# taintpro98/rnd-semantic-segmentation

Measured on AMD Instinct MI355X. Metric: train images/sec at 769x769 bf16 (DeepLabV2-ResNet101 + ASPP), higher is better.
Workload: dtype bf16; 1 GPU; train_src.py DeepLabV2-R101 bf16, 769x769 synthetic Cityscapes crops, batch 8 per GPU, 1xMI355X; global_batch=8, parallelism=dp1, weights=formula (synthetic), hip_graph_replay=False

## Files before the change

include/mi355seg.h:

```cpp
#ifndef MI355SEG_H
#define MI355SEG_H

#include <stddef.h>
#include <stdint.h>

#ifdef __cplusplus
extern "C" {
#endif

#define MI355SEG_VERSION 100

#define MI_OK 0
#define MI_EINVAL (-22)
#define MI_ENOMEM (-12)
#define MI_EHIP (-5)

#define MI_EPI_SCALE_BIAS 1
#define MI_EPI_RESIDUAL 2
#define MI_EPI_RELU 4
#define MI_EPI_MASK 8
#define MI_EPI_OUT_F32 16
#define MI_EPI_ZSPLIT 32
#define MI_EPI_WRITE_MASK 64
#define MI_EPI_LEAKY 256
// ... 63 lines not shown
int mi_upsample_ac_fwd(const float* low, float* up, int B, int h, int w, int K, int H, int W, void* stream);
int mi_upsample_ac_bwd(const float* dup, float* dlow, int B, int h, int w, int K, int H, int W, void* stream);

size_t mi_ce_workspace(int B, int H, int W);
int mi_softmax_ce_fwd(const float* logits, const int64_t* labels, float* loss_out ,
                      int B, int K, int H, int W, int ignore_index, void* workspace, size_t workspace_bytes, void* stream);
int mi_softmax_ce_bwd(const float* logits, const int64_t* labels, const float* loss_out, float* dlogits,
                      int B, int K, int H, int W, int ignore_index, float grad_scale, void* stream);

size_t mi_upsample_ce_workspace(int B, int h, int w, int K, int H, int W);
int mi_upsample_ce(const float* low, const int64_t* labels, float* loss_out , float* dlow,
                   int B, int h, int w, int K, int H, int W, int ignore_index, float grad_scale,
                   void* workspace, size_t workspace_bytes, void* stream);

int mi_upsample_ce_ex(const float* low, const int64_t* labels, float* loss_out , float* dlow,
                      int B, int h, int w, int K, int H, int W, int ignore_index, float grad_scale, int align_corners,
                      void* workspace, size_t workspace_bytes, void* stream);

int mi_upsample_softmax(const float* low, float* probs, uint8_t* pred, int B, int h, int w, int K, int H, int W, void* stream);

typedef struct { const float* low; int h, w; int mirror; } MiProbSource;
int mi_upsample_softmax_multi(const MiProbSource* src, int n, float* probs, int K, int H, int W, float div_a, float div_b, void* stream);

int mi_image_resize_ac(const float* x, float* out, int B, int C, int H, int W, int Ho, int Wo, int with_mirror, void* stream);

int mi_sgd_step(float* p, const float* g, float* buf, size_t n, float lr, float momentum, float weight_decay, void* stream);
int mi_sgd_step_dev(float* p, const float* g, float* buf, size_t n, const float* hyper , void* stream);

int mi_stem_pool_fwd(const void* y, const float* scale, const float* shift, void* pool, uint8_t* idx,
                     int B, int Hc, int Wc, int C, int Hp, int Wp, void* stream);
int mi_stem_pool_bwd(const void* dpool, const uint8_t* idx, const float* scale, void* dy,
                     int B, int Hc, int Wc, int C, int Hp, int Wp, void* stream);
int mi_stem_im2col(const void* x_bf16_nhwc, void* col_bf16, int B, int H, int W, int Ho, int Wo, int ncols, void* stream);

int mi_bias_grad_bf16(const void* dy_bf16, float* db, int M, int N, int accumulate,
                      void* workspace , size_t workspace_bytes, void* stream);
size_t mi_upsample_softce_workspace(int B, int h, int w, int K, int H, int W);
int mi_upsample_softce(const float* seg_low, float inv_temperature, float clip, const float* d_low, int ldD, int domain,
                       float* loss_out, float* dd_low, int B, int h, int w, int K, int H, int W, float grad_scale,
                       void* workspace, size_t workspace_bytes, void* stream);
size_t mi_upsample_softce_2grid_workspace(int B, int hd, int wd, int K, int H, int W);
int mi_upsample_softce_2grid(const float* seg_low, int hs, int ws, int seg_align_corners, float inv_temperature, float clip,
                             const float* d_low, int hd, int wd, int ldD, int d_align_corners, int domain, float grad_scale,
                             float* loss_out, float* dd_low, int B, int K, int H, int W, void* workspace, size_t workspace_bytes, void* stream);
int mi_adam_step(float* p, const float* g, float* exp_avg, float* exp_avg_sq, size_t n, float lr, float beta1, float beta2,
                 float eps, int step, void* stream);
int mi_adam_step_clamped(float* p, float* g, float* exp_avg, float* exp_avg_sq, size_t n, float lr, float beta1, float beta2,
                         float eps, int step, float grad_clamp, void* stream);

int mi_adam_step_dev(float* p, float* g, float* exp_avg, float* exp_avg_sq, size_t n, const float* hyper , void* stream);

int mi_pack_weight_f32(const float* w_oihw, float* wp, int O, int I, int ksize, void* stream);
int mi_conv_f32(const float* a, const float* wp, float* out, int B, int Ha, int Wa, int Ca, int Ho, int Wo, int N,
                int ksize, int stride, int pad, int dil, const float* scale, const float* bias, const float* res,
                int flags, void* stream);
int mi_stem_f32(const float* x_nchw, const float* w, const float* scale, const float* shift, float* y_nhwc,
                int B, int H, int W, void* stream);
int mi_maxpool_f32(const float* y_nhwc, float* pool_nhwc, int B, int Hc, int Wc, int C, void* stream);

int mi_comm_unique_id(void* id128 );
int mi_comm_init_rank(void** comm , int nranks, const void* id128 , int rank);
int mi_comm_destroy(void* comm);
int mi_allreduce_bucket(void* ptr, size_t count, int dtype, int average, void* comm, void* stream);

int mi_relu_mask(const void* x_bf16, const void* msk, void* y_bf16, size_t n, int bits, void* stream);
int mi_frozen_bn_fold(const float* w, const float* b, const float* mean, const float* var, float* scale, float* shift, int n, void* stream);
// ... 129 lines not shown
```

rnd_semantic_segmentation_amd/_lib.py:

```python
import ctypes
import os

import torch
from ctypes import c_char_p, c_double, c_float, c_int, c_long, c_size_t, c_void_p

_HERE = os.path.dirname(os.path.abspath(__file__))
LIB_PATH = os.environ.get("MI355SEG_LIB") or os.path.join(_HERE, "libmi355seg.so")
HEADER_PATH = os.path.join(os.path.dirname(_HERE), "include", "mi355seg.h")

P, I, F, Z, L = c_void_p, c_int, c_float, c_size_t, c_long

SIGNATURES = {
    "mi_version": (I, []),
    "mi_last_error": (c_char_p, []),
    "mi_pack_weight_fwd": (I, [P, P, I, I, I, P]),
    "mi_pack_weight_dgrad": (I, [P, P, P, I, I, I, P]),
    "mi_pack_weights_multi": (I, [P, P, P, P, P, I, I, P]),
    "mi_conv_gemm": (I, [P, P, P] + [I] * 12 + [P, P, P, P, P, I, I, F, P]),
    "mi_conv_gemm_route": (I, [I] * 10),
    "mi_conv_gemm_pp": (I, [P, P, P] + [I] * 12 + [P, P, P, P, P, I, I, F, I, P]),
    "mi_conv_chain": (I, [P] * 6 + [L, I, I, I] + [P] * 8 + [I, I, P]),
    "mi_conv_wgrad_workspace": (Z, [I] * 6),
    "mi_conv_wgrad_route": (I, [I] * 12),
    "mi_conv_wgrad": (I, [P, P, P] + [I] * 11 + [P, I, I, I, Z, P, Z, P]),
    "mi_conv_wgrad_job_bytes": (Z, []),
    "mi_conv_wgrad_partial": (I, [P, P, P] + [I] * 11 + [P, I, I, I, Z, P, Z, P, P]),
    "mi_conv_wgrad_reduce": (I, [P, I, P]),
    "mi_aspp_pack_fwd": (I, [P, P, I, I, P]),
    "mi_aspp_pack_dgrad": (I, [P, P, I, I, P]),
    "mi_aspp_col2im": (I, [P, P, P, I, I, I, I, P, P]),
    "mi_aspp_im2col": (I, [P, P, I, I, I, I, P, P]),
    "mi_colsum_workspace": (Z, [I, I]),
    "mi_aspp_bias_grad": (I, [P, P, I, I, I, P, Z, P]),
    "mi_upsample_ac_fwd": (I, [P, P] + [I] * 6 + [P]),
    "mi_upsample_ac_bwd": (I, [P, P] + [I] * 6 + [P]),
    "mi_ce_workspace": (Z, [I, I, I]),
    "mi_softmax_ce_fwd": (I, [P, P, P, I, I, I, I, I, P, Z, P]),
    "mi_softmax_ce_bwd": (I, [P, P, P, P, I, I, I, I, I, F, P]),
    "mi_upsample_ce_workspace": (Z, [I] * 6),
    "mi_upsample_ce": (I, [P, P, P, P] + [I] * 7 + [F, P, Z, P]),
    "mi_upsample_ce_ex": (I, [P, P, P, P] + [I] * 7 + [F, I, P, Z, P]),
    "mi_upsample_softmax": (I, [P, P, P] + [I] * 6 + [P]),
    "mi_upsample_softmax_multi": (I, [P, I, P, I, I, I, F, F, P]),
    "mi_image_resize_ac": (I, [P, P] + [I] * 7 + [P]),
    "mi_stem_pool_fwd": (I, [P, P, P, P, P] + [I] * 6 + [P]),
    "mi_stem_pool_bwd": (I, [P, P, P, P] + [I] * 6 + [P]),
    "mi_stem_im2col": (I, [P, P] + [I] * 6 + [P]),
    "mi_bias_grad_bf16": (I, [P, P, I, I, I, P, Z, P]),
    "mi_upsample_softce_workspace": (Z, [I] * 6),
    "mi_upsample_softce": (I, [P, F, F, P, I, I, P, P] + [I] * 6 + [F, P, Z, P]),
    "mi_upsample_softce_2grid_workspace": (Z, [I] * 6),
    "mi_upsample_softce_2grid": (I, [P, I, I, I, F, F, P, I, I, I, I, I, F, P, P, I, I, I, I, P, Z, P]),
    "mi_adam_step": (I, [P, P, P, P, Z, F, F, F, F, I, P]),
    "mi_adam_step_clamped": (I, [P, P, P, P, Z, F, F, F, F, I, F, P]),
    "mi_adam_step_dev": (I, [P, P, P, P, Z, P, P]),
    "mi_sgd_step": (I, [P, P, P, Z, F, F, F, P]),
    "mi_sgd_step_dev": (I, [P, P, P, Z, P, P]),
    "mi_pack_weight_f32": (I, [P, P, I, I, I, P]),
    "mi_conv_f32": (I, [P, P, P] + [I] * 11 + [P, P, P, I, P]),
    "mi_stem_f32": (I, [P, P, P, P, P, I, I, I, P]),
    "mi_maxpool_f32": (I, [P, P, I, I, I, I, P]),
    "mi_comm_unique_id": (I, [P]),
    "mi_comm_init_rank": (I, [P, I, P, I]),
    "mi_comm_destroy": (I, [P]),
    "mi_allreduce_bucket": (I, [P, Z, I, I, P, P]),
    "mi_relu_mask": (I, [P, P, P, Z, I, P]),
    "mi_frozen_bn_fold": (I, [P, P, P, P, P, P, I, P]),
    "mi_structure_loss_workspace": (Z, [I, I, I]),
    "mi_structure_loss": (I, [P, P, I, I, I, P, P, F, P, Z, P]),
    "mi_bn_workspace": (Z, [L, I]),
    "mi_bn_colsum": (I, [P, P, L, I, P, P, Z, P]),
    "mi_bn_apply": (I, [P, P, P, P, P, P, P, I, L, I, P]),
    "mi_bn_colsum2": (I, [P, P, L, I, P, P, P, Z, P]),
    "mi_conv_gemm_stats_workspace": (Z, [L, I]),
    "mi_conv_gemm_stats": (I, [P, P, P] + [I] * 11 + [P, P, P, Z, P, P, P, P, P, F, F, P, P]),
    "mi_bn_finalize": (I, [P, P, P, c_double, P, P, P, P, P, F, F, P, I, P]),
    "mi_bn_bwd_colsums": (I, [P, P, P, P, P, L, I, P, P, P, Z, P]),
    "mi_bn_bwd_apply": (I, [P, P, P, P, P, P, P, F, P, P, L, I, P]),
    "mi_gconv_pack_elems": (Z, [I] * 4),
    "mi_gconv_pack_multi": (I, [P, P, P, P, I, I, P]),
# ... 84 lines not shown
```

rnd_semantic_segmentation_amd/csrc/stem.hip:

```cpp
#include "mi_common.h"

namespace {

__global__ void stem_pool_fwd_kernel(const bf16x8* __restrict__ y, const float* __restrict__ scale, const float* __restrict__ shift,
                                     bf16x8* __restrict__ pool, uint8_t* __restrict__ idx, int B, int Hc, int Wc, int C8, int Hp, int Wp) {
    const long id = (long)blockIdx.x * blockDim.x + threadIdx.x;
    if (id >= (long)B * Hp * Wp * C8) return;
    const int c8 = (int)(id % C8);
    const int wo = (int)((id / C8) % Wp), ho = (int)((id / ((long)C8 * Wp)) % Hp), b = (int)(id / ((long)C8 * Wp * Hp));
    float sc[8], sh[8], best[8];
    int bi[8];
#pragma unroll
    for (int e = 0; e < 8; ++e) {
        sc[e] = scale[c8 * 8 + e];
        sh[e] = shift[c8 * 8 + e];
        best[e] = -3.0e38f;
        bi[e] = 9;
    }
#pragma unroll
    for (int ky = 0; ky < 3; ++ky) {
        const int h = 2 * ho - 1 + ky;
        if ((unsigned)h >= (unsigned)Hc) continue;
#pragma unroll
        for (int kx = 0; kx < 3; ++kx) {
// ... 88 lines not shown
    const __bf16* img = x + (long)b * H * W * 3;
    bf16x8 v;
#pragma unroll
    for (int e = 0; e < 8; ++e) {
        __bf16 val = (__bf16)0.f;
        if (k + e < 147) {
            const int h = 2 * ho - 3 + ky, w = 2 * wo - 3 + kx;
            if ((unsigned)h < (unsigned)H && (unsigned)w < (unsigned)W) val = img[((long)h * W + w) * 3 + c];
        }
        v[e] = val;
        if (++kx == 7) {
            kx = 0;
            if (++ky == 7) {
                ky = 0;
                ++c;
            }
        }
    }
    col[((long)blockIdx.y * Wo + wo) * groups + kg] = v;
}
}

extern "C" int mi_stem_im2col(const void* x_bf16_nhwc, void* col_bf16, int B, int H, int W, int Ho, int Wo, int ncols, void* stream) {
    MI_REQUIRE(x_bf16_nhwc && col_bf16 && B > 0 && H > 0 && W > 0, "mi_stem_im2col: bad argument");
    MI_REQUIRE(ncols >= 152 && ncols % 8 == 0 && ncols <= 256, "mi_stem_im2col: ncols=%d (a multiple of 8 in [152, 256])", ncols);
    MI_REQUIRE(Ho == (H + 6 - 7) / 2 + 1 && Wo == (W + 6 - 7) / 2 + 1, "mi_stem_im2col: output size must be that of a 7x7/2/3 conv");
    MI_REQUIRE(mi_aligned16(col_bf16), "mi_stem_im2col: alignment");
    MI_REQUIRE((long)B * Ho < 65536, "mi_stem_im2col: B * Ho = %ld exceeds the grid", (long)B * Ho);
    hipLaunchKernelGGL(stem_im2col_kernel, dim3((unsigned)((Wo * (ncols / 8) + 255) / 256), (unsigned)(B * Ho)), dim3(256), 0, (hipStream_t)stream,
                       (const __bf16*)x_bf16_nhwc, (bf16x8*)col_bf16, B, H, W, Ho, Wo, ncols / 8);
    MI_CHECK_LAUNCH("mi_stem_im2col");
    return MI_OK;
}
```

rnd_semantic_segmentation_amd/host/engine.py:

```python
import contextlib
import os

import torch

from .. import kernels as K
from . import arch


class FlatStore:

    ALIGN = 64

    def __init__(self, named_params, device):
        self.names = [n for n, _ in named_params]
        self.params = [p for _, p in named_params]
        self.offsets = []
        off = 0
        for p in self.params:
            self.offsets.append(off)
            off += -(-p.numel() // self.ALIGN) * self.ALIGN
        self.total = off
        self.data = torch.zeros(off, dtype=torch.float32, device=device)
        self.grad = torch.zeros(off, dtype=torch.float32, device=device)
        self.written = set()
# ... 577 lines not shown
            self._sig = sig

    def forward(self, x):
        self.prepare()
        h, w = x.shape[1], x.shape[2]
        out = None
        for wp, b, d in zip(self._wp, self._b, self.rates):
            out = K.conv_f32(x, wp, (h, w), 3, 1, d, d, bias=b, res=out)
        return out


def stem_conv_forward(x, weight):
    y, col = K.stem_conv_fwd(x, weight)
    return y, (col,)


def stem_conv_wgrad(dy_nhwc, saved):
    return K.stem_wgrad(dy_nhwc, col=saved[0])


class StemConvFn(torch.autograd.Function):

    @staticmethod
    def forward(ctx, x, weight):
        y, saved = stem_conv_forward(x, weight)
        ctx.save_for_backward(*saved)
        return y

    @staticmethod
    def backward(ctx, dy):
        return None, stem_conv_wgrad(dy.contiguous(), ctx.saved_tensors)


class StemFn(torch.autograd.Function):

    @staticmethod
    def forward(ctx, x, weight, scale, shift):
        y, saved = stem_conv_forward(x, weight)
        pool, idx = K.stem_pool_fwd(y, scale, shift)
        ctx.save_for_backward(idx, scale, *saved)
        ctx.conv_hw = (y.shape[1], y.shape[2])
        return pool

    @staticmethod
    def backward(ctx, dpool):
        idx, scale = ctx.saved_tensors[:2]
        dy = K.stem_pool_bwd(dpool.contiguous(), idx, scale, ctx.conv_hw)
        return None, stem_conv_wgrad(dy, ctx.saved_tensors[2:]), None, None


class StagesFn(torch.autograd.Function):

    @staticmethod
    def forward(ctx, x, eng, *weights):
        train = any(ctx.needs_input_grad)
        eng.prepare(train)
        feat, saved, fbits = eng.forward(x, save=train)
        ctx.eng, ctx.saved, ctx.fbits = eng, saved, fbits
        return feat

    @staticmethod
    def backward(ctx, dfeat):
        dfeat = dfeat.contiguous()
        dx = ctx.eng.backward(ctx.saved, ctx.fbits, dfeat, ctx.needs_input_grad[0])
        ctx.saved = ctx.fbits = None
        return (dx, None) + (None,) * (len(ctx.needs_input_grad) - 2)


class AsppEngine:

    def __init__(self, owner, rates, num_classes, in_channels):
        self.owner, self.rates, self.K, self.C = owner, tuple(int(r) for r in rates), num_classes, in_channels
        self.wall = self.wallT = None
        self._sig = None
        self._have_dgrad = False

    def _w4(self):
        ws = [getattr(self.owner.conv2d_list, str(i)).weight for i in range(4)]
        n = ws[0].numel()
# ... 143 lines not shown
```

rnd_semantic_segmentation_amd/host/modules.py:

```python
import logging
import os

import torch
import torch.nn as nn
import torch.nn.functional as F

from .. import _lib
from . import arch, engine


class FrozenBatchNorm2d(nn.Module):

    def __init__(self, n):
        super().__init__()
        self.register_buffer("weight", torch.ones(n))
        self.register_buffer("bias", torch.zeros(n))
        self.register_buffer("running_mean", torch.zeros(n))
        self.register_buffer("running_var", torch.ones(n))

    def fold(self):
        scale = self.weight * self.running_var.rsqrt()
        return scale, self.bias - self.running_mean * scale

    def forward(self, x):
# ... 65 lines not shown

    def engine_parameters(self):
        return [(k, p) for k, p in self.named_parameters()]

    def ensure_flat(self):
        dev = self.backbone.conv1.weight.device
        if self._store is None or not self._store.intact() or self._store.data.device != dev:
            self._store = engine.FlatStore(self.engine_parameters(), dev)
        return self._store

    def _stem_fold(self):
        bn = self.backbone.bn1
        sig = (engine.bn_versions(bn), bn.weight.data_ptr())
        if getattr(self, "_stem_sig", None) != sig:
            self._stem_scale, self._stem_shift = engine.bn_fold(bn)
            self._stem_sig = sig
        return self._stem_scale, self._stem_shift

    def sync_batchnorm(self, on=True):
        for m in self.backbone.modules():
            if isinstance(m, nn.BatchNorm2d):
                m._mi_sync = bool(on)
        return self

    def forward(self, x):
        _require_gpu(x, "resnet_feature_extractor")
        if self.precision == "fp32":
            if torch.is_grad_enabled() and any(p.requires_grad for p in self.parameters()):
                raise _lib.MiError("the fp32 path is forward-only (evaluation): call it under torch.no_grad(), or "
                                   "set_precision('bf16') to train")
            return self._fp32.forward(x.float()).permute(0, 3, 1, 2)
        self.ensure_flat()
        bb = self.backbone
        xb = x.to(dtype=torch.bfloat16).contiguous(memory_format=torch.channels_last)
        self._engine.batch_stats = (not self.freeze_bn) and self.training
        if self._engine.batch_stats:
            y = engine.BnStemFn.apply(xb, bb.conv1.weight, bb.bn1.weight, bb.bn1.bias, bb.bn1)
            params = [p for rt in self._engine.convs for p in (rt.weight, rt.bn.weight, rt.bn.bias)]
            return engine.BnStagesFn.apply(y, self._engine, *params).permute(0, 3, 1, 2)
        scale, shift = self._stem_fold()
        y = engine.StemFn.apply(xb, bb.conv1.weight, scale, shift)
        weights = [rt.weight for rt in self._engine.convs]
        feat = engine.StagesFn.apply(y, self._engine, *weights)
        return feat.permute(0, 3, 1, 2)


class ASPP_Classifier_V2(nn.Module):

    def __init__(self, in_channels, dilation_series, padding_series, num_classes):
        super().__init__()
        if list(dilation_series) != list(padding_series) or len(dilation_series) != 4:
            raise NotImplementedError("ASPP engine expects 4 branches with padding == dilation (build.py:26-28 passes "
                                      "[6, 12, 18, 24] twice)")
        self.in_channels, self.num_classes = in_channels, num_classes
        self.rates = tuple(int(d) for d in dilation_series)
        self.conv2d_list = arch.Holder()
        for i in range(4):
            node = arch.Holder()
            node.weight = nn.Parameter(torch.randn(num_classes, in_channels, 3, 3) * 0.01)
            self.conv2d_list.add_module(str(i), node)
        bound = 1.0 / (in_channels * 9) ** 0.5
        for i in range(4):
            getattr(self.conv2d_list, str(i)).bias = nn.Parameter(torch.empty(num_classes).uniform_(-bound, bound))
        self._engine = engine.AsppEngine(self, self.rates, num_classes, in_channels)
        self._fp32 = engine.Fp32Aspp(self, self.rates)
        self.precision = "bf16"
        self._store = None

    def set_precision(self, precision):
        if precision not in ("bf16", "fp32"):
            raise ValueError("precision %r (bf16 | fp32)" % (precision,))
        self.precision = precision
        return self

# ... 105 lines not shown
```

rnd_semantic_segmentation_amd/kernels.py:

```python
import ctypes

import torch

from . import _lib
from ._lib import check

EPI_SCALE_BIAS, EPI_RESIDUAL, EPI_RELU, EPI_MASK, EPI_OUT_F32, EPI_ZSPLIT, EPI_WRITE_MASK, EPI_BITMASK, EPI_LEAKY = 1, 2, 4, 8, 16, 32, 64, 128, 256
GATHER_FWD, GATHER_DGRAD = 0, 1
ASPP_ZGW, ASPP_KPAD = 20, 704


def _stream():
    return ctypes.c_void_p(torch.cuda.current_stream().cuda_stream)


PROFILE = None


def _timed(name, flops, launch, tag=None):
    if PROFILE is None:
        return launch()
    e0, e1 = torch.cuda.Event(enable_timing=True), torch.cuda.Event(enable_timing=True)
    e0.record()
    rc = launch()
# ... 413 lines not shown

def stem_im2col(x, ncols):
    _chk_dtype = x.dtype
    if _chk_dtype != torch.bfloat16 or not x.is_cuda:
        raise _lib.MiError("stem_im2col: x must be a bf16 GPU tensor")
    B, _, H, W = x.shape
    Ho, Wo = (H + 6 - 7) // 2 + 1, (W + 6 - 7) // 2 + 1
    xn = x.permute(0, 2, 3, 1)
    if not xn.is_contiguous():
        xn = xn.contiguous()
    col = torch.empty((B, Ho, Wo, ncols), dtype=torch.bfloat16, device=x.device)
    check(_lib.lib().mi_stem_im2col(_p(xn), _p(col), B, H, W, Ho, Wo, ncols, _stream()), "mi_stem_im2col")
    return col


def stem_conv_fwd(x, weight):
    col = stem_im2col(x, 192)
    O = weight.shape[0]
    wp = torch.zeros((1, O, 192), dtype=torch.bfloat16, device=x.device)
    wp[0, :, :147] = weight.detach().reshape(O, 147).to(torch.bfloat16)
    return conv_gemm(col, wp, (col.shape[1], col.shape[2]), 1, 1, 0, 1, GATHER_FWD), col


def stem_wgrad(dy, x=None, col=None):
    _chk(dy, torch.bfloat16, "dy")
    if col is None:
        col = stem_im2col(x, 160)
    O, n = dy.shape[-1], col.shape[-1]
    dw = torch.empty((O, n, 1, 1), dtype=torch.float32, device=dy.device)
    conv_wgrad(dy, col, dw, 1, 1, 0, 1)
    return dw.view(O, n)[:, :147].reshape(O, 3, 7, 7)


def bias_grad_bf16(dy, db, accumulate=False):
    _chk(dy, torch.bfloat16, "dy")
    _chk(db, torch.float32, "db")
    N = dy.shape[-1]
    L = _lib.lib()
    ws = _workspace(L.mi_colsum_workspace(dy.numel() // N, N), dy.device, "colsum")
    check(L.mi_bias_grad_bf16(_p(dy), _p(db), dy.numel() // N, N, int(accumulate), _p(ws), ws.numel(), _stream()), "mi_bias_grad_bf16")
    return db


def upsample_softce(seg_low, d_low, size, domain, temperature=1.8, clip=0.9, want_grad=True, grad_scale=1.0):
    _chk(seg_low, torch.float32, "seg_low")
    _chk(d_low, torch.float32, "d_low")
    B, h, w, Kc = seg_low.shape
    ldD = d_low.shape[-1]
    H, W = size
    L = _lib.lib()
    ws = _workspace(L.mi_upsample_softce_workspace(B, h, w, Kc, H, W), seg_low.device, "softce")
    out = torch.empty(2, dtype=torch.float32, device=seg_low.device)
    dd = torch.empty_like(d_low) if want_grad else None
    check(L.mi_upsample_softce(_p(seg_low), 1.0 / float(temperature), float(clip), _p(d_low), ldD, int(domain), _p(out), _p(dd), B, h, w, Kc,
                               H, W, float(grad_scale), _p(ws), ws.numel(), _stream()), "mi_upsample_softce")
    return out, dd


def upsample_softce_2grid(seg_low, d_low, size, domain, temperature=1.8, clip=0.9, want_grad=True, grad_scale=1.0, seg_align_corners=False,
                          d_align_corners=True):
    _chk(seg_low, torch.float32, "seg_low")
    _chk(d_low, torch.float32, "d_low")
    B, hs, ws, Kc = seg_low.shape
    Bd, hd, wd, ldD = d_low.shape
    if Bd != B:
        raise _lib.MiError("upsample_softce_2grid: seg_low holds %d images, d_low %d" % (B, Bd))
# ... 238 lines not shown
```

Measured before the change: 298.6 images/s.

## Fuse stem conv, BN, ReLU and max-pool forward, and pool-backward with wgrad

Adds a forward stem kernel that loads an image window, runs the 7x7/2 conv with MFMA, applies the folded BN scale/shift and ReLU, and max-pools in LDS. The conv output never goes to global memory and no im2col buffer is built. The backward kernel rebuilds dy from dpool and the pool indices per tile and computes the weight gradient directly against the image, with a per-workgroup partial reduction. It reads fp32 NCHW input directly, skipping the bf16 channels_last conversion. This removes large intermediate tensors and several launches at the stem, at the cost of complex hand-tiled kernels.

```diff
diff --git a/include/mi355seg.h b/include/mi355seg.h
--- a/include/mi355seg.h
+++ b/include/mi355seg.h
@@ -119,6 +119,11 @@
 int mi_stem_pool_bwd(const void* dpool, const uint8_t* idx, const float* scale, void* dy,
                      int B, int Hc, int Wc, int C, int Hp, int Wp, void* stream);
 int mi_stem_im2col(const void* x_bf16_nhwc, void* col_bf16, int B, int H, int W, int Ho, int Wo, int ncols, void* stream);
+int mi_stem_fwd_fused(const void* x, int x_is_f32_nchw, const float* w, const float* scale, const float* shift, void* pool, uint8_t* idx,
+                      int B, int H, int W, int C, int Hp, int Wp, void* stream);
+size_t mi_stem_wgrad_fused_workspace(void);
+int mi_stem_wgrad_fused(const void* dpool, const uint8_t* idx, const float* scale, const void* x, int x_is_f32_nchw, float* dw,
+                        int B, int H, int W, int C, int Hp, int Wp, void* workspace, size_t workspace_bytes, void* stream);
 
 int mi_bias_grad_bf16(const void* dy_bf16, float* db, int M, int N, int accumulate,
                       void* workspace , size_t workspace_bytes, void* stream);
diff --git a/rnd_semantic_segmentation_amd/_lib.py b/rnd_semantic_segmentation_amd/_lib.py
--- a/rnd_semantic_segmentation_amd/_lib.py
+++ b/rnd_semantic_segmentation_amd/_lib.py
@@ -46,6 +46,9 @@
     "mi_stem_pool_fwd": (I, [P, P, P, P, P] + [I] * 6 + [P]),
     "mi_stem_pool_bwd": (I, [P, P, P, P] + [I] * 6 + [P]),
     "mi_stem_im2col": (I, [P, P] + [I] * 6 + [P]),
+    "mi_stem_fwd_fused": (I, [P, I, P, P, P, P, P] + [I] * 6 + [P]),
+    "mi_stem_wgrad_fused_workspace": (Z, []),
+    "mi_stem_wgrad_fused": (I, [P, P, P, P, I, P] + [I] * 6 + [P, Z, P]),
     "mi_bias_grad_bf16": (I, [P, P, I, I, I, P, Z, P]),
     "mi_upsample_softce_workspace": (Z, [I] * 6),
     "mi_upsample_softce": (I, [P, F, F, P, I, I, P, P] + [I] * 6 + [F, P, Z, P]),
diff --git a/rnd_semantic_segmentation_amd/csrc/stem.hip b/rnd_semantic_segmentation_amd/csrc/stem.hip
--- a/rnd_semantic_segmentation_amd/csrc/stem.hip
+++ b/rnd_semantic_segmentation_amd/csrc/stem.hip
@@ -144,3 +144,401 @@
     MI_CHECK_LAUNCH("mi_stem_im2col");
     return MI_OK;
 }
+
+namespace {
+constexpr int SF_NC = 17;
+constexpr int SF_NPIX = SF_NC * SF_NC;
+constexpr int SF_MT = (SF_NPIX + 15) / 16;
+constexpr int SF_WIN = 2 * (SF_NC - 1) + 7;
+constexpr int SF_IMG_ELEMS = 3 * SF_WIN * SF_WIN;
+constexpr int SF_IMG_BYTES = (SF_IMG_ELEMS * 2 + 15) / 16 * 16;
+constexpr int SF_NLD = (SF_IMG_ELEMS + 255) / 256;
+constexpr int SF_CSTRIDE = 144;
+constexpr int SF_CONV_BYTES = SF_NPIX * SF_CSTRIDE;
+constexpr int SF_WROW = 168;
+constexpr int SF_LDS = SF_IMG_BYTES + SF_CONV_BYTES + 512;
+static_assert(64 * SF_WROW * 2 <= SF_CONV_BYTES, "the staged weights must fit the conv tile");
+
+template <bool F32IN> __device__ __forceinline__ __bf16 stem_pixel(const void* x, int b, int c, int h, int w, int H, int W) {
+    if (F32IN) return (__bf16) reinterpret_cast<const float*>(x)[(unsigned)(((b * 3 + c) * H + h) * W + w)];
+    return reinterpret_cast<const __bf16*>(x)[(unsigned)(((b * H + h) * W + w) * 3 + c)];
+}
+
+template <bool F32IN>
+__global__ __launch_bounds__(256, 2) void stem_fwd_fused_kernel(const void* __restrict__ x, const float* __restrict__ w, const float* __restrict__ scale,
+                                                                const float* __restrict__ shift, bf16x8* __restrict__ pool, uint8_t* __restrict__ idx,
+                                                                int H, int W, int Hc, int Wc, int Hp, int Wp, int tiles_x, int tiles_y, int ntiles) {
+    __shared__ __attribute__((aligned(16))) char smem[SF_LDS];
+    __bf16* img = reinterpret_cast<__bf16*>(smem);
+    char* cbuf = smem + SF_IMG_BYTES;
+    float* aff = reinterpret_cast<float*>(smem + SF_IMG_BYTES + SF_CONV_BYTES);
+    const int tid = threadIdx.x, lane = tid & 63, wave = tid >> 6;
+    const int frow = lane & 15, fq = lane >> 4;
+
+    {
+        __bf16* wl = reinterpret_cast<__bf16*>(cbuf);
+        for (int e = tid; e < 64 * 160; e += 256) {
+            const int n = e / 160, k = e - n * 160;
+            wl[n * SF_WROW + k] = (__bf16)(k < 147 ? w[n * 147 + k] : 0.f);
+        }
+        if (tid < 64) aff[tid] = scale[tid];
+        else if (tid < 128) aff[tid] = shift[tid - 64];
+    }
+    __syncthreads();
+    bf16x8 wf[5][4];
+#pragma unroll
+    for (int kb = 0; kb < 5; ++kb)
+#pragma unroll
+        for (int nt = 0; nt < 4; ++nt)
+            wf[kb][nt] = *reinterpret_cast<const bf16x8*>(cbuf + ((nt * 16 + frow) * SF_WROW + kb * 32 + fq * 8) * 2);
+    int koff[5][8];
+#pragma unroll
+    for (int kb = 0; kb < 5; ++kb)
+#pragma unroll
+        for (int j = 0; j < 8; ++j) {
+            const int k = kb * 32 + fq * 8 + j, kk = k < 147 ? k : 0;
+            const int c = kk / 49, r = kk - c * 49, ky = r / 7, kx = r - ky * 7;
+            koff[kb][j] = (c * SF_WIN + ky) * SF_WIN + kx + 2 * frow + wave * (2 * SF_WIN);
+        }
+
+    __bf16 win[SF_NLD];
+    auto load_window = [&](int t) {
+        const int tx = t % tiles_x, ty = (t / tiles_x) % tiles_y, b = t / (tiles_x * tiles_y);
+        const int r0 = 2 * (2 * ty * 8 - 1) - 3, c0 = 2 * (2 * tx * 8 - 1) - 3;
+        int tl = tid;
+        asm volatile("" : "+v"(tl));
+#pragma unroll
+        for (int i = 0; i < SF_NLD; ++i) {
+            const int e = tl + i * 256;
+            const int c = e / (SF_WIN * SF_WIN), rem = e - c * (SF_WIN * SF_WIN);
+            const int r = rem / SF_WIN, col = rem - r * SF_WIN;
+            const int h = r0 + r, ww = c0 + col;
+            const bool ok = e < SF_IMG_ELEMS && (unsigned)h < (unsigned)H && (unsigned)ww < (unsigned)W;
+            const __bf16 v = stem_pixel<F32IN>(x, ok ? b : 0, ok ? c : 0, ok ? h : 0, ok ? ww : 0, H, W);
+            win[i] = ok ? v : (__bf16)0.f;
+        }
+    };
+    if ((int)blockIdx.x < ntiles) load_window(blockIdx.x);
+    for (int t = blockIdx.x; t < ntiles; t += gridDim.x) {
+        const int tx = t % tiles_x, ty = (t / tiles_x) % tiles_y, b = t / (tiles_x * tiles_y);
+        const int ho0 = ty * 8, wo0 = tx * 8;
+        const int hc0 = 2 * ho0 - 1, wc0 = 2 * wo0 - 1;
+#pragma unroll
+        for (int i = 0; i < SF_NLD; ++i)
+            if (tid + i * 256 < SF_IMG_ELEMS) img[tid + i * 256] = win[i];
+        __syncthreads();
+
+        auto conv_tile = [&](int delta, int m, bool live) {
+            f32x4 acc[4];
+#pragma unroll
+            for (int nt = 0; nt < 4; ++nt) acc[nt] = f32x4{0.f, 0.f, 0.f, 0.f};
+#pragma unroll
+            for (int kb = 0; kb < 5; ++kb) {
+                bf16x8 pf;
+#pragma unroll
+                for (int j = 0; j < 8; ++j) {
+                    __bf16 v = img[koff[kb][j] + delta];
+                    if (kb == 4 && kb * 32 + fq * 8 + j >= 147) v = (__bf16)0.f;
+                    pf[j] = v;
+                }
+#pragma unroll
+                for (int nt = 0; nt < 4; ++nt) acc[nt] = __builtin_amdgcn_mfma_f32_16x16x32_bf16(wf[kb][nt], pf, acc[nt], 0, 0, 0);
+            }
+            if (live) {
+#pragma unroll
+                for (int nt = 0; nt < 4; ++nt) {
+                    const int n = nt * 16 + fq * 4;
+                    const f32x4 sc = *reinterpret_cast<const f32x4*>(aff + n), sh = *reinterpret_cast<const f32x4*>(aff + 64 + n);
+                    bf16x4 o;
+#pragma unroll
+                    for (int r = 0; r < 4; ++r) {
+                        float f = (float)(__bf16)acc[nt][r] * sc[r] + sh[r];
+                        o[r] = (__bf16)(f > 0.f ? f : 0.f);
+                    }
+                    *reinterpret_cast<bf16x4*>(cbuf + m * SF_CSTRIDE + n * 2) = o;
+                }
+            }
+        };
+#pragma unroll
+        for (int i = 0; i < 5; ++i)
+            if (wave + 4 * i < SF_NC) conv_tile(i * (8 * SF_WIN), (wave + 4 * i) * SF_NC + frow, true);
+        if (wave == 1 || wave == 2) {
+            const int h0 = (wave - 1) * 16 + frow, hl = h0 < SF_NC ? h0 : SF_NC - 1;
+            conv_tile((hl - wave) * (2 * SF_WIN) + 2 * (16 - frow), hl * SF_NC + 16, h0 < SF_NC);
+        }
+        __syncthreads();
+        if (t + (int)gridDim.x < ntiles) load_window(t + gridDim.x);
+
+        const int pp = tid >> 2, cq = tid & 3;
+        const int ph = pp >> 3, pw = pp & 7;
+        const int ho = ho0 + ph, wo = wo0 + pw;
+        if (ho < Hp && wo < Wp) {
+            const long pix = ((long)b * Hp + ho) * Wp + wo;
+            u32x4 ibytes;
+#pragma unroll
+            for (int half = 0; half < 2; ++half) {
+                const int c8 = cq * 2 + half;
+                uint32_t best[8];
+#pragma unroll
+                for (int e = 0; e < 8; ++e) best[e] = 0u;
+#pragma unroll
+                for (int ky = 0; ky < 3; ++ky) {
+                    const int hl = 2 * ph + ky;
+                    if ((unsigned)(hc0 + hl) >= (unsigned)Hc) continue;
+#pragma unroll
+                    for (int kx = 0; kx < 3; ++kx) {
+                        const int wl = 2 * pw + kx;
+                        if ((unsigned)(wc0 + wl) >= (unsigned)Wc) continue;
+                        const u32x4 v = *reinterpret_cast<const u32x4*>(cbuf + (hl * SF_NC + wl) * SF_CSTRIDE + c8 * 16);
+                        const uint32_t code = 8u - (uint32_t)(ky * 3 + kx);
+#pragma unroll
+                        for (int d = 0; d < 4; ++d) {
+                            const uint32_t lo = (v[d] << 16) | code, hi = (v[d] & 0xffff0000u) | code;
+                            best[2 * d] = lo > best[2 * d] ? lo : best[2 * d];
+                            best[2 * d + 1] = hi > best[2 * d + 1] ? hi : best[2 * d + 1];
+                        }
+                    }
+                }
+                u32x4 o;
+                uint32_t lo = 0, hi = 0;
+#pragma unroll
+                for (int e = 0; e < 8; ++e) {
+                    const uint32_t byte = (best[e] >> 16) ? 8u - (best[e] & 15u) : 9u;
+                    if (e < 4) lo |= byte << (8 * e);
+                    else hi |= byte << (8 * (e - 4));
+                }
+#pragma unroll
+                for (int d = 0; d < 4; ++d) o[d] = (best[2 * d] >> 16) | (best[2 * d + 1] & 0xffff0000u);
+                *reinterpret_cast<u32x4*>(pool + pix * 8 + c8) = o;
+                ibytes[half * 2] = lo;
+                ibytes[half * 2 + 1] = hi;
+            }
+            *reinterpret_cast<u32x4*>(idx + pix * 64 + cq * 16) = ibytes;
+        }
+    }
+}
+
+constexpr int SW_R = 5, SW_SEG = 32;
+constexpr int SW_WR = 2 * SW_R + 5, SW_WC = 70;
+constexpr int SW_IMG_ELEMS = 3 * SW_WR * SW_WC;
+constexpr int SW_IMG_BYTES = (SW_IMG_ELEMS * 2 + 15) / 16 * 16;
+constexpr int SW_DROW = 80;
+constexpr int SW_DY_BYTES = SW_R * 64 * SW_DROW;
+constexpr int SW_THREADS = 320;
+constexpr int SW_PH = 4, SW_PW = 17, SW_PPIX = SW_PH * SW_PW;
+constexpr int SW_PL_BYTES = SW_PPIX * (128 + 64);
+constexpr int SW_NLD = (SW_IMG_ELEMS + SW_THREADS - 1) / SW_THREADS;
+constexpr int SW_NCH = (SW_PPIX * 12 + SW_THREADS - 1) / SW_THREADS;
+constexpr int SW_MAX_WG = 512;
+static_assert(SW_R * SW_SEG * 8 % SW_THREADS == 0, "dy items split evenly over the threads");
+
+template <bool F32IN>
+__global__ __launch_bounds__(SW_THREADS) void stem_wgrad_fused_kernel(const bf16x8* __restrict__ dpool, const uint8_t* __restrict__ idx,
+                                                                       const float* __restrict__ scale, const void* __restrict__ x,
+                                                                       float* __restrict__ part, int H, int W, int Hc, int Wc, int Hp, int Wp,
+                                                                       int units_y, int units_x, long units) {
+    __shared__ __attribute__((aligned(16))) char smem[SW_IMG_BYTES + SW_DY_BYTES + SW_PL_BYTES];
+    __bf16* img = reinterpret_cast<__bf16*>(smem);
+    char* dyt = smem + SW_IMG_BYTES;
+    char* pl = dyt + SW_DY_BYTES;
+    const int tid = threadIdx.x, lane = tid & 63, wave = tid >> 6;
+    const int frow = lane & 15, fq = lane >> 4;
+    int koff[2];
+#pragma unroll
+    for (int i = 0; i < 2; ++i) {
+        const int k = (wave * 2 + i) * 16 + frow, kk = k < 147 ? k : 0;
+        const int c = kk / 49, r = kk - c * 49, ky = r / 7, kx = r - ky * 7;
+        koff[i] = (c * SW_WR + ky) * SW_WC + kx + 16 * fq;
+    }
+    f32x4 acc[4][2];
+#pragma unroll
+    for (int ot = 0; ot < 4; ++ot)
+#pragma unroll
+        for (int i = 0; i < 2; ++i) acc[ot][i] = f32x4{0.f, 0.f, 0.f, 0.f};
+    int arow[4];
+#pragma unroll
+    for (int ot = 0; ot < 4; ++ot) arow[ot] = ((frow & 7) * 8 + ot * 2 + (frow >> 3)) * SW_DROW + fq * 16;
+
+    __bf16 win[SW_NLD];
+    u32x4 pch[SW_NCH];
+    auto load_unit = [&](long u) {
+        const int ux = (int)(u % units_x), uy = (int)((u / units_x) % units_y), b = (int)(u / ((long)units_x * units_y));
+        const int hc0 = uy * SW_R, wc0 = ux * SW_SEG;
+        const int r0 = 2 * hc0 - 3, c0 = 2 * wc0 - 3;
+        int tl = tid;
+        asm volatile("" : "+v"(tl));
+#pragma unroll
+        for (int i = 0; i < SW_NLD; ++i) {
+            const int e = tl + i * SW_THREADS;
+            const int c = e / (SW_WR * SW_WC), rem = e - c * (SW_WR * SW_WC);
+            const int r = rem / SW_WC, col = rem - r * SW_WC;
+            const int h = r0 + r, ww = c0 + col;
+            const bool ok = e < SW_IMG_ELEMS && col < SW_WC - 1 && (unsigned)h < (unsigned)H && (unsigned)ww < (unsigned)W;
+            const __bf16 v = stem_pixel<F32IN>(x, ok ? b : 0, ok ? c : 0, ok ? h : 0, ok ? ww : 0, H, W);
+            win[i] = ok ? v : (__bf16)0.f;
+        }
+        const int hob = hc0 >> 1, wob = wc0 >> 1;
+#pragma unroll
+        for (int i = 0; i < SW_NCH; ++i) {
+            const int id = tl + i * SW_THREADS;
+            const bool isg = id < SW_PPIX * 8;
+            const int pix = isg ? id >> 3 : (id - SW_PPIX * 8) >> 2, sub = isg ? id & 7 : (id - SW_PPIX * 8) & 3;
+            const int pr = pix / SW_PW, pc = pix - pr * SW_PW;
+            const bool ok = id < SW_PPIX * 12 && hob + pr < Hp && wob + pc < Wp;
+            const unsigned p = ok ? (unsigned)((b * Hp + hob + pr) * Wp + wob + pc) : 0u;
+            const u32x4* src = isg ? reinterpret_cast<const u32x4*>(dpool) + p * 8 + sub : reinterpret_cast<const u32x4*>(idx) + p * 4 + sub;
+            pch[i] = *src;
+        }
+    };
+    const long u0 = units * blockIdx.x / gridDim.x, u1 = units * (blockIdx.x + 1) / gridDim.x;
+    if (u0 < u1) load_unit(u0);
+    for (long u = u0; u < u1; ++u) {
+        const int ux = (int)(u % units_x), uy = (int)((u / units_x) % units_y);
+        const int hc0 = uy * SW_R, wc0 = ux * SW_SEG;
+        const int hob = hc0 >> 1, wob = wc0 >> 1;
+        __syncthreads();
+#pragma unroll
+        for (int i = 0; i < SW_NLD; ++i)
+            if (tid + i * SW_THREADS < SW_IMG_ELEMS) img[tid + i * SW_THREADS] = win[i];
+#pragma unroll
+        for (int i = 0; i < SW_NCH; ++i)
+            if (tid + i * SW_THREADS < SW_PPIX * 12) *reinterpret_cast<u32x4*>(pl + (tid + i * SW_THREADS) * 16) = pch[i];
+        __syncthreads();
+        if (u + 1 < u1) load_unit(u + 1);
+        for (int it = tid; it < SW_R * SW_SEG * 8; it += SW_THREADS) {
+            const int c8 = it & 7, px = 2 * ((it >> 3) & 15) + ((it >> 7) & 1), rl = it >> 8;
+            const int h = hc0 + rl, ww = wc0 + px;
+            float a[8] = {0.f, 0.f, 0.f, 0.f, 0.f, 0.f, 0.f, 0.f};
+            if (h < Hc && ww < Wc) {
+                const int ho_lo = h >> 1, ho_hi = (h + 1) >> 1, wo_lo = ww >> 1, wo_hi = (ww + 1) >> 1;
+                for (int ho = ho_lo; ho <= ho_hi; ++ho) {
+                    if (ho >= Hp) continue;
+                    const int ky = h - (2 * ho - 1);
+                    for (int wo = wo_lo; wo <= wo_hi; ++wo) {
+                        if (wo >= Wp) continue;
+                        const int tap = ky * 3 + (ww - (2 * wo - 1));
+                        const int pix = (ho - hob) * SW_PW + (wo - wob);
+                        const bf16x8 g = *reinterpret_cast<const bf16x8*>(pl + (pix * 8 + c8) * 16);
+                        const uint2 ib = *reinterpret_cast<const uint2*>(pl + SW_PPIX * 128 + (pix * 8 + c8) * 8);
+#pragma unroll
+                        for (int e = 0; e < 8; ++e) {
+                            const unsigned byte = ((e < 4 ? ib.x : ib.y) >> (8 * (e & 3))) & 0xffu;
+                            if ((int)byte == tap) a[e] += (float)g[e];
+                        }
+                    }
+                }
+            }
+            __bf16* drow = reinterpret_cast<__bf16*>(dyt + rl * (64 * SW_DROW)) + px;
+#pragma unroll
+            for (int e = 0; e < 8; ++e) drow[(e * 8 + c8) * (SW_DROW / 2)] = (__bf16)(a[e] * scale[c8 * 8 + e]);
+        }
+        __syncthreads();
+#pragma unroll
+        for (int rl = 0; rl < SW_R; ++rl) {
+            bf16x8 af[4], pf[2];
+#pragma unroll
+            for (int ot = 0; ot < 4; ++ot) af[ot] = *reinterpret_cast<const bf16x8*>(dyt + rl * (64 * SW_DROW) + arow[ot]);
+#pragma unroll
+            for (int i = 0; i < 2; ++i) {
+                const __bf16* src = img + koff[i] + 2 * rl * SW_WC;
+#pragma unroll
+                for (int j = 0; j < 8; ++j) pf[i][j] = src[2 * j];
+            }
+#pragma unroll
+            for (int ot = 0; ot < 4; ++ot)
+#pragma unroll
+                for (int i = 0; i < 2; ++i) acc[ot][i] = __builtin_amdgcn_mfma_f32_16x16x32_bf16(af[ot], pf[i], acc[ot][i], 0, 0, 0);
+        }
+    }
+    float* plane = part + (long)blockIdx.x * (64 * 160);
+#pragma unroll
+    for (int ot = 0; ot < 4; ++ot)
+#pragma unroll
+        for (int i = 0; i < 2; ++i) *reinterpret_cast<f32x4*>(plane + ((wave * 2 + i) * 16 + frow) * 64 + ot * 16 + fq * 4) = acc[ot][i];
+}
+
+__global__ __launch_bounds__(256) void stem_wgrad_reduce_kernel(const float* __restrict__ part, float* __restrict__ dw, int nparts) {
+    __shared__ float sums[16][16];
+    const int li = threadIdx.x & 15, s = threadIdx.x >> 4;
+    const int i = blockIdx.x * 16 + li;
+    const int k = i >> 6, o = i & 63;
+    const int per = (nparts + 15) / 16, g0 = s * per, g1 = g0 + per < nparts ? g0 + per : nparts;
+    const float* src = part + i;
+    float a = 0.f;
+    int g = g0;
+    for (; g + 8 <= g1; g += 8) {
+        float v[8];
+#pragma unroll
+        for (int q = 0; q < 8; ++q) v[q] = src[(long)(g + q) * (64 * 160)];
+#pragma unroll
+        for (int q = 0; q < 8; ++q) a += v[q];
+    }
+    for (; g < g1; ++g) a += src[(long)g * (64 * 160)];
+    sums[s][li] = a;
+    __syncthreads();
+    if (s == 0) {
+        float t = sums[0][li];
+#pragma unroll
+        for (int q = 1; q < 16; ++q) t += sums[q][li];
+        dw[o * 147 + k] = t;
+    }
+}
+
+inline bool stem_fused_sizes_ok(int B, int H, int W, int Hp, int Wp, int& Hc, int& Wc) {
+    Hc = (H + 6 - 7) / 2 + 1;
+    Wc = (W + 6 - 7) / 2 + 1;
+    return Hp == (Hc + 2 - 3) / 2 + 1 && Wp == (Wc + 2 - 3) / 2 + 1 && (long)B * H * W * 3 < (1L << 31) && (long)B * Hc * Wc * 64 < (1L << 31);
+}
+inline int stem_wgrad_units(int B, int Hc, int Wc, int& uy, int& ux) {
+    uy = (Hc + SW_R - 1) / SW_R;
+    ux = (Wc + SW_SEG - 1) / SW_SEG;
+    return B * uy * ux;
+}
+}
+
+extern "C" int mi_stem_fwd_fused(const void* x, int x_is_f32_nchw, const float* w, const float* scale, const float* shift, void* pool, uint8_t* idx,
+                                 int B, int H, int W, int C, int Hp, int Wp, void* stream) {
+    MI_REQUIRE(x && w && scale && shift && pool && idx && B > 0 && H > 0 && W > 0, "mi_stem_fwd_fused: bad argument");
+    MI_REQUIRE(C == 64, "mi_stem_fwd_fused: C=%d (the stem has 64 output channels)", C);
+    int Hc, Wc;
+    MI_REQUIRE(stem_fused_sizes_ok(B, H, W, Hp, Wp, Hc, Wc), "mi_stem_fwd_fused: pooled size must be that of a 7x7/2/3 conv + 3x3/2/1 max-pool, 32-bit element counts");
+    MI_REQUIRE(mi_aligned16(pool) && mi_aligned16(idx), "mi_stem_fwd_fused: alignment");
+    const int tiles_x = (Wp + 7) / 8, tiles_y = (Hp + 7) / 8;
+    const long ntiles = (long)B * tiles_x * tiles_y;
+    MI_REQUIRE(ntiles < (1L << 31), "mi_stem_fwd_fused: too many tiles");
+    const unsigned grid = (unsigned)(ntiles < 512 ? ntiles : 512);
+    if (x_is_f32_nchw)
+        hipLaunchKernelGGL(stem_fwd_fused_kernel<true>, dim3(grid), dim3(256), 0, (hipStream_t)stream, x, w, scale, shift, (bf16x8*)pool, idx, H, W, Hc, Wc,
+                           Hp, Wp, tiles_x, tiles_y, (int)ntiles);
+    else
+        hipLaunchKernelGGL(stem_fwd_fused_kernel<false>, dim3(grid), dim3(256), 0, (hipStream_t)stream, x, w, scale, shift, (bf16x8*)pool, idx, H, W, Hc,
+                           Wc, Hp, Wp, tiles_x, tiles_y, (int)ntiles);
+    MI_CHECK_LAUNCH("mi_stem_fwd_fused");
+    return MI_OK;
+}
+
+extern "C" size_t mi_stem_wgrad_fused_workspace(void) { return (size_t)SW_MAX_WG * 64 * 160 * sizeof(float); }
+
+extern "C" int mi_stem_wgrad_fused(const void* dpool, const uint8_t* idx, const float* scale, const void* x, int x_is_f32_nchw, float* dw, int B, int H,
+                                   int W, int C, int Hp, int Wp, void* workspace, size_t workspace_bytes, void* stream) {
+    MI_REQUIRE(dpool && idx && scale && x && dw && workspace && B > 0 && H > 0 && W > 0, "mi_stem_wgrad_fused: bad argument");
+    MI_REQUIRE(C == 64, "mi_stem_wgrad_fused: C=%d (the stem has 64 output channels)", C);
+    int Hc, Wc;
+    MI_REQUIRE(stem_fused_sizes_ok(B, H, W, Hp, Wp, Hc, Wc), "mi_stem_wgrad_fused: pooled size must be that of a 7x7/2/3 conv + 3x3/2/1 max-pool, 32-bit element counts");
+    MI_REQUIRE(mi_aligned16(dpool) && mi_aligned16(idx) && mi_aligned16(workspace), "mi_stem_wgrad_fused: alignment");
+    MI_REQUIRE(workspace_bytes >= mi_stem_wgrad_fused_workspace(), "mi_stem_wgrad_fused: workspace of %zu bytes, need %zu", workspace_bytes,
+               mi_stem_wgrad_fused_workspace());
+    int uy, ux;
+    const long units = stem_wgrad_units(B, Hc, Wc, uy, ux);
+    const int nwg = (int)(units < SW_MAX_WG ? units : SW_MAX_WG);
+    if (x_is_f32_nchw)
+        hipLaunchKernelGGL(stem_wgrad_fused_kernel<true>, dim3(nwg), dim3(SW_THREADS), 0, (hipStream_t)stream, (const bf16x8*)dpool, idx, scale, x,
+                           (float*)workspace, H, W, Hc, Wc, Hp, Wp, uy, ux, units);
+    else
+        hipLaunchKernelGGL(stem_wgrad_fused_kernel<false>, dim3(nwg), dim3(SW_THREADS), 0, (hipStream_t)stream, (const bf16x8*)dpool, idx, scale, x,
+                           (float*)workspace, H, W, Hc, Wc, Hp, Wp, uy, ux, units);
+    MI_CHECK_LAUNCH("mi_stem_wgrad_fused");
+    hipLaunchKernelGGL(stem_wgrad_reduce_kernel, dim3(64 * 147 / 16), dim3(256), 0, (hipStream_t)stream, (const float*)workspace, dw, nwg);
+    MI_CHECK_LAUNCH("mi_stem_wgrad_fused (reduce)");
+    return MI_OK;
+}
diff --git a/rnd_semantic_segmentation_amd/host/engine.py b/rnd_semantic_segmentation_amd/host/engine.py
--- a/rnd_semantic_segmentation_amd/host/engine.py
+++ b/rnd_semantic_segmentation_amd/host/engine.py
@@ -633,11 +633,27 @@
         return None, stem_conv_wgrad(dy.contiguous(), ctx.saved_tensors)
 
 
+def stem_fused_on():
+    return os.environ.get("MI_STEM_FUSED", "1") != "0"
+
+
+def stem_image(x):
+    if stem_fused_on() and ((x.dtype == torch.float32 and x.is_contiguous()) or
+                            (x.dtype == torch.bfloat16 and x.is_contiguous(memory_format=torch.channels_last))):
+        return x
+    return x.to(dtype=torch.bfloat16).contiguous(memory_format=torch.channels_last)
+
+
 class StemFn(torch.autograd.Function):
 
     @staticmethod
     def forward(ctx, x, weight, scale, shift):
-        y, saved = stem_conv_forward(x, weight)
+        ctx.fused = stem_fused_on()
+        if ctx.fused:
+            pool, idx = K.stem_fwd_fused(x, weight.detach(), scale, shift)
+            ctx.save_for_backward(idx, scale, x)
+            return pool
+        y, saved = stem_conv_forward(stem_image(x), weight)
         pool, idx = K.stem_pool_fwd(y, scale, shift)
         ctx.save_for_backward(idx, scale, *saved)
         ctx.conv_hw = (y.shape[1], y.shape[2])
@@ -646,6 +662,8 @@
     @staticmethod
     def backward(ctx, dpool):
         idx, scale = ctx.saved_tensors[:2]
+        if ctx.fused:
+            return None, K.stem_wgrad_fused(dpool.contiguous(), idx, scale, ctx.saved_tensors[2]), None, None
         dy = K.stem_pool_bwd(dpool.contiguous(), idx, scale, ctx.conv_hw)
         return None, stem_conv_wgrad(dy, ctx.saved_tensors[2:]), None, None
 
diff --git a/rnd_semantic_segmentation_amd/host/modules.py b/rnd_semantic_segmentation_amd/host/modules.py
--- a/rnd_semantic_segmentation_amd/host/modules.py
+++ b/rnd_semantic_segmentation_amd/host/modules.py
@@ -121,14 +121,14 @@
             return self._fp32.forward(x.float()).permute(0, 3, 1, 2)
         self.ensure_flat()
         bb = self.backbone
-        xb = x.to(dtype=torch.bfloat16).contiguous(memory_format=torch.channels_last)
         self._engine.batch_stats = (not self.freeze_bn) and self.training
         if self._engine.batch_stats:
+            xb = x.to(dtype=torch.bfloat16).contiguous(memory_format=torch.channels_last)
             y = engine.BnStemFn.apply(xb, bb.conv1.weight, bb.bn1.weight, bb.bn1.bias, bb.bn1)
             params = [p for rt in self._engine.convs for p in (rt.weight, rt.bn.weight, rt.bn.bias)]
             return engine.BnStagesFn.apply(y, self._engine, *params).permute(0, 3, 1, 2)
         scale, shift = self._stem_fold()
-        y = engine.StemFn.apply(xb, bb.conv1.weight, scale, shift)
+        y = engine.StemFn.apply(engine.stem_image(x), bb.conv1.weight, scale, shift)
         weights = [rt.weight for rt in self._engine.convs]
         feat = engine.StagesFn.apply(y, self._engine, *weights)
         return feat.permute(0, 3, 1, 2)
diff --git a/rnd_semantic_segmentation_amd/kernels.py b/rnd_semantic_segmentation_amd/kernels.py
--- a/rnd_semantic_segmentation_amd/kernels.py
+++ b/rnd_semantic_segmentation_amd/kernels.py
@@ -469,6 +469,52 @@
     return dw.view(O, n)[:, :147].reshape(O, 3, 7, 7)
 
 
+def _stem_image(x, name):
+    if not x.is_cuda or x.dim() != 4 or x.shape[1] != 3:
+        raise _lib.MiError("%s: x must be a [B,3,H,W] GPU tensor" % name)
+    if x.dtype == torch.float32 and x.is_contiguous():
+        return 1
+    if x.dtype == torch.bfloat16 and x.permute(0, 2, 3, 1).is_contiguous():
+        return 0
+    raise _lib.MiError("%s: x must be fp32 NCHW contiguous or bf16 channels_last" % name)
+
+
+def stem_fwd_fused(x, weight, scale, shift):
+    f32 = _stem_image(x, "stem_fwd_fused")
+    _chk(weight, torch.float32, "weight")
+    _chk(scale, torch.float32, "scale")
+    _chk(shift, torch.float32, "shift")
+    B, _, H, W = x.shape
+    O = weight.shape[0]
+    if tuple(weight.shape[1:]) != (3, 7, 7) or scale.numel() != O or shift.numel() != O:
+        raise _lib.MiError("stem_fwd_fused: weight %s must be [O,3,7,7] with O scales and shifts" % (tuple(weight.shape),))
+    Hc, Wc = (H - 1) // 2 + 1, (W - 1) // 2 + 1
+    Hp, Wp = (Hc - 1) // 2 + 1, (Wc - 1) // 2 + 1
+    pool = torch.empty((B, Hp, Wp, O), dtype=torch.bfloat16, device=x.device)
+    idx = torch.empty((B, Hp, Wp, O), dtype=torch.uint8, device=x.device)
+    check(_lib.lib().mi_stem_fwd_fused(_p(x), f32, _p(weight), _p(scale), _p(shift), _p(pool), _p(idx), B, H, W, O, Hp, Wp, _stream()),
+          "mi_stem_fwd_fused")
+    return pool, idx
+
+
+def stem_wgrad_fused(dpool, idx, scale, x):
+    f32 = _stem_image(x, "stem_wgrad_fused")
+    _chk(dpool, torch.bfloat16, "dpool")
+    _chk(idx, torch.uint8, "idx")
+    _chk(scale, torch.float32, "scale")
+    B, _, H, W = x.shape
+    _, Hp, Wp, O = dpool.shape
+    if idx.shape != dpool.shape or dpool.shape[0] != B or scale.numel() != O:
+        raise _lib.MiError("stem_wgrad_fused: dpool %s, idx %s, scale %s and x %s do not belong together" %
+                           (tuple(dpool.shape), tuple(idx.shape), tuple(scale.shape), tuple(x.shape)))
+    L = _lib.lib()
+    ws = _workspace(L.mi_stem_wgrad_fused_workspace(), dpool.device, "stem_wgrad")
+    dw = torch.empty((O, 3, 7, 7), dtype=torch.float32, device=dpool.device)
+    check(L.mi_stem_wgrad_fused(_p(dpool), _p(idx), _p(scale), _p(x), f32, _p(dw), B, H, W, O, Hp, Wp, _p(ws), ws.numel(), _stream()),
+          "mi_stem_wgrad_fused")
+    return dw
+
+
 def bias_grad_bf16(dy, db, accumulate=False):
     _chk(dy, torch.bfloat16, "dy")
     _chk(db, torch.float32, "db")
```

After: 300.9 images/s (median of 6 runs). About the same (+0.8%).
